# CAMMA-public/SelfPose3d

Hardware: AMD Instinct MI355X
Metric: multi-view samples/sec (5-view Panoptic, 80x80x20 voxel) (higher is better)
Workload: dtype f32

## Files before the change

include/sp3d.h:

```cpp
#ifndef SP3D_H
#define SP3D_H

#include <stdint.h>

#ifdef __cplusplus
extern "C" {
#endif

#define SP3D_ABI_VERSION 3
#define SP3D_MAX_VIEWS 16
#define SP3D_MAX_TOPK 32

#define SP3D_CAM_STRIDE 64
#define SP3D_CAM_R 0
#define SP3D_CAM_T 9
#define SP3D_CAM_F 12
#define SP3D_CAM_C 14
#define SP3D_CAM_K 16
#define SP3D_CAM_P 19
#define SP3D_CAM_A 21
#define SP3D_CAM_W0 27
#define SP3D_CAM_H0 28
#define SP3D_CAM_FLIP 29
#define SP3D_CAM_RXY 32
// ... 90 lines not shown
                                 const float *grid_size, int W_in, int H_in, void *stream);

int sp3d_unproject_one_bwd(const float *cam, const int32_t *sample_of, const float *centers, const uint8_t *valid,
                           const float *grad_cubes, int64_t grad_cube_stride, const uint16_t *pass_mask, float *grad_hm,
                           int B, int P, int V, int h, int w, int X, int Y, int Z, const float *grid_size, int W_in,
                           int H_in, void *stream);

int sp3d_unproject_one_bwd_det(const float *cam, const int32_t *sample_of, const float *centers, const uint8_t *valid,
                               const float *grad_cubes, int64_t grad_cube_stride, const uint16_t *pass_mask,
                               int64_t *grad_fixed, const float *scale, int B, int P, int V, int h, int w, int X, int Y,
                               int Z, const float *grid_size, int W_in, int H_in, void *stream);

int64_t sp3d_nms_topk_workspace_bytes(int B, int X, int Y, int Z, int k);
int sp3d_nms_topk(const float *root_cubes, int B, int X, int Y, int Z, int k, const float *grid_size,
                  const float *grid_center, float *vals, int64_t *idx, float *locs, void *workspace, void *stream);
int sp3d_nms_proposals(const float *root_cubes, int B, int X, int Y, int Z, int k, const float *grid_size,
                       const float *grid_center, float threshold, float *vals, int64_t *idx, float *locs,
                       float *grid_centers, void *workspace, void *stream);

int sp3d_soft_argmax(const float *x, const float *grids, float *out, int Bv, int J, int64_t N, float beta,
                     void *stream);
int sp3d_soft_argmax_grid(const float *x, const float *centers, const float *grid_size, int X, int Y, int Z,
                          float *out, int Bv, int J, float beta, void *stream);
int sp3d_soft_argmax_grid_train(const float *x, const float *centers, const float *grid_size, int X, int Y, int Z, float *out,
                                float *stats, int Bv, int J, float beta, void *stream);
int sp3d_soft_argmax_grid_bwd(const float *x, const float *centers, const float *grid_size, int X, int Y, int Z,
                              const float *out, const float *stats, const float *grad_out, float *grad_x, int Bv, int J,
                              float beta, void *stream);

int sp3d_channel_shift_act(float *y, const float *shift, const float *residual, int mode, int64_t batch, int C,
                           int64_t inner, int channels_last, void *stream);

int sp3d_fetch_ring(const float *ring, float *dst, uint32_t *counter, int R, int n, void *stream);

int sp3d_maxpool2x_cl(const float *x, float *y, int B, int X, int Y, int Z, int C, void *stream);

int sp3d_crop_shift_act_cl(const float *src, float *dst, const float *shift, int B, int C, int X, int Y, int Z, int SX, int SY,
                           int SZ, int relu, void *stream);

int sp3d_rfft3d(const float *in, float *out, int batch, int SX, int SY, int SZ, void *stream);
int sp3d_irfft3d(float *in, float *out, int batch, int SX, int SY, int SZ, void *stream);

int sp3d_cfft2d(float *data, int batch, int SX, int SY, int inverse, void *stream);
int sp3d_cfft2d_ex(float *data, int batch, int SX, int SY, int inverse, int rows_in, int rows_out, void *stream);

int sp3d_zdft_fwd_cl(const float *x, float *spec, int B, int C, int Cout, int X, int Y, int Z, int SX, int SY, int SZ,
                     void *stream);
int sp3d_zdft_inv_cl(const float *spec, float *y, const float *shift, int B, int O, int X, int Y, int Z, int SX, int SY, int SZ,
                     int relu, void *stream);

int sp3d_unproject_fwd_zdft(const float *const *hm_views, int Jp, const float *cam, const float *centers,
                            const uint8_t *valid, float *spec, int B, int V, int J, int h, int w, int X, int Y, int Z,
                            const float grid_size[3], int W_in, int H_in, int SZ, void *stream);
int sp3d_cfft2d_88_tiled(const float *tiled, float *planes, int batch, int X, int Y, void *stream);

int sp3d_freq_contract_ty(const float *X, const float *T, const float *tw, float *Y, int B, int C, int O, int rows, int SY,
                          void *stream);

int sp3d_gaussian_target_3d(const float *roots, int B, int R, const float *gx, const float *gy, const float *gz, int X,
                            int Y, int Z, float sigma, float *target, void *stream);
int sp3d_render_root_heatmaps(const float *roots, int B, int R, const float *cam, int V, int h, int w, float stride,
                              float *out, void *stream);
int sp3d_render_joints_fwd(const float *kps, const int *count, int N, int P, int J, int h, int w, float sigma, float *out,
                           void *stream);
int sp3d_render_joints_bwd(const float *kps, const int *count, const float *grad_out, int N, int P, int J, int h, int w,
                           float sigma, float *grad_kps, void *stream);

int sp3d_freq_contract(const float *X, const float *W, float *Y, int B, int C, int O, int64_t F, void *stream);
int sp3d_freq_contract_ex(const float *P, const float *Q, float *Y, int I, int J, int K, int64_t F, int64_t sPi,
                          int64_t sPk, int64_t sQj, int64_t sQk, int conj_p, int conj_q, void *stream);

int sp3d_wino_input(const float *x, float *V, int B, int X, int Y, int Z, int C, void *stream);
int sp3d_wino_output(const float *M, float *y, const float *shift, const float *residual, int mode, int B, int X, int Y,
                     int Z, int O, void *stream);
int sp3d_wino_fused(const float *x, const float *U, float *y, const float *shift, const float *residual, int mode, int B,
                    int X, int Y, int Z, int C, int O, void *stream);

int sp3d_wino_fused_split(const float *x, const void *U3, float *y, const float *shift, const float *residual, int mode, int B,
                          int X, int Y, int Z, int C, int O, void *stream);

int sp3d_wino_fused_split64(const float *x, const void *U3, float *y, const float *shift, const float *residual, int mode,
                            int B, int X, int Y, int Z, int C, int O, void *stream);

int sp3d_conv3_split(const float *x, const void *W3, float *y, const float *shift, const float *residual, int mode, int B,
                     int X, int Y, int Z, int C, int O, void *stream);


int sp3d_conv3_split_skip(const float *x, const void *W3, float *y, const float *shift, const float *xs, const void *WS,
                          int B, int X, int Y, int Z, int C, int O, int CS, void *stream);

int sp3d_wino_fused_split64_skip(const float *x, const void *U3, float *y, const float *shift, const float *xs, const void *WS,
                                 int B, int X, int Y, int Z, int C, int O, int CS, void *stream);

int sp3d_upsample2x_scatter(const float *G, float *out, const float *shift, const float *skip, int64_t batch, int X, int Y,
                            int Z, int O, void *stream);

int sp3d_upsample2x_scatter_head(const float *G, float *head, const float *shift, const float *skip, const float *wout,
                                 const float *bout, int64_t batch, int X, int Y, int Z, int O, int J, void *stream);

int sp3d_upconv2x_fused(const float *x, const void *w_split, const float *shift, const float *skip, const float *w_out,
                        const float *b_out, float *out, int64_t batch, int X, int Y, int Z, int CIN, int O, int J, void *stream);

#define SP3D_GBN_F32 0
#define SP3D_GBN_F64 1
#define SP3D_GBN_REPLICAS 16
#define SP3D_GBN_PLAIN 0
#define SP3D_GBN_RELU 1
#define SP3D_GBN_ADD_RELU 2
int64_t sp3d_gbn_workspace_bytes(int G, int C);
int sp3d_gbn_forward(const void *x, void *y, int dtype, const int32_t *group_of, const int32_t *group_samples, int N,
                     int64_t S, int C, int G, int G_update, const void *weight, const void *bias, void *running_mean,
                     void *running_var, double eps, double momentum, int mode, const void *residual, void *mean,
                     void *invstd, void *scale, void *shift, double *workspace, void *stream);
int sp3d_gbn_backward(const void *x, const void *dy, void *dx, int dtype, const int32_t *group_of,
                      const int32_t *group_samples, int N, int64_t S, int C, int G, const void *weight, const void *mean,
                      const void *invstd, const void *scale, const void *shift, int mode, const void *y,
                      void *grad_residual, void *grad_weight, void *grad_bias, void *k123, double *workspace, void *stream);

#ifdef __cplusplus
}
#endif
#endif
```

selfpose3d_amd/_lib.py:

```python
from __future__ import annotations

import ctypes as C
import os
from typing import Optional, Sequence

import torch

_HERE = os.path.dirname(os.path.abspath(__file__))
_DEFAULT_LIB_PATH = os.path.join(_HERE, "libsp3d.so")
NOPK_LIB_PATH = os.path.join(_HERE, "libsp3d_nopk.so")
LIB_PATH = os.environ.get("SP3D_LIB_PATH") or _DEFAULT_LIB_PATH

LAYOUT_PLANAR = 0
LAYOUT_NHWC = 1
OUT_CHANNELS_LAST = 0x100
HM_BF16 = 0x200
OUT_BF16 = 0x400
HM_ONE_CHANNEL = 0x800
HM_WIDE_MASK = 0x1000
SCATTER_AUTO, SCATTER_PER_TAP, SCATTER_MERGE = 0, 2, 3
SCATTER_WIDE = 0x100
MAX_VIEWS = 16
MAX_TOPK = 32
ABI_VERSION = 3
# ... 711 lines not shown
    Fn = 1
    for d in Pf.shape[2:]:
        Fn *= int(d)
    p0, p1, q0, q1 = int(Pf.shape[0]), int(Pf.shape[1]), int(Qf.shape[0]), int(Qf.shape[1])
    if mode == "fwd":
        I, K, J = p0, p1, q0
        sPi, sPk, sQj, sQk, cp, cq = p1 * Fn, Fn, q1 * Fn, Fn, 0, 1
        ok = q1 == p1
    elif mode == "dx":
        I, K, J = p0, p1, q1
        sPi, sPk, sQj, sQk, cp, cq = p1 * Fn, Fn, Fn, q1 * Fn, 0, 0
        ok = q0 == p1
    elif mode == "dw":
        I, K, J = p1, p0, q1
        sPi, sPk, sQj, sQk, cp, cq = Fn, p1 * Fn, Fn, q1 * Fn, 1, 0
        ok = q0 == p0
    else:
        raise Sp3dError(f"freq_contract_ex: unknown mode {mode}")
    if not ok:
        raise Sp3dError("freq_contract_ex: contracted dimensions differ")
    Y = torch.empty((I, J) + tuple(Pf.shape[2:]), dtype=torch.complex64, device=Pf.device)
    check(lib.sp3d_freq_contract_ex(Pf.data_ptr(), Qf.data_ptr(), Y.data_ptr(), I, J, K, Fn, sPi, sPk, sQj, sQk, cp, cq,
                                    _stream(Pf.device)), "sp3d_freq_contract_ex")
    return Y


_WINO_G = ((1.0, 0.0, 0.0), (0.5, 0.5, 0.5), (0.5, -0.5, 0.5), (0.0, 0.0, 1.0))


def wino_weights(w: torch.Tensor) -> torch.Tensor:
    G = torch.tensor(_WINO_G, dtype=torch.float64, device=w.device)
    u = torch.einsum("ai,bj,ck,ozijk->abczo", G, G, G, w.double())
    return u.reshape(64, w.shape[1], w.shape[0]).float().contiguous()


def wino_weights_split(U: torch.Tensor, chunk: int = 8) -> torch.Tensor:
    P, Cc, O = (int(v) for v in U.shape)
    U = U.float()
    hi = U.bfloat16()
    r = U - hi.float()
    mid = r.bfloat16()
    lo = (r - mid.float()).bfloat16()
    pieces = torch.stack([mid, hi, lo], 0).reshape(3, P, Cc // chunk, chunk // 4, 4, O)
    return pieces.permute(1, 2, 3, 5, 0, 4).contiguous()


def conv_weights_split(w: torch.Tensor) -> torch.Tensor:
    O, Cc = int(w.shape[0]), int(w.shape[1])
    taps = int(w.shape[2]) * int(w.shape[3]) * int(w.shape[4])
    pc = wino_weights_split(w.float().permute(4, 3, 2, 1, 0).reshape(taps, Cc, O).contiguous(), 8)
    mid, hi, lo = pc[..., 0, :], pc[..., 1, :], pc[..., 2, :]
    return torch.stack([hi, lo, hi, hi, mid, mid], -2).contiguous()


def conv_weights_split24(w: torch.Tensor) -> torch.Tensor:
    O, Cc = int(w.shape[0]), int(w.shape[1])
    pc = wino_weights_split(w.float().permute(4, 3, 2, 1, 0).reshape(27, Cc, O).contiguous(), 8)
    pc = pc.reshape(27, Cc // 8, 2, O // 32, 32, 3, 4).permute(0, 1, 3, 2, 4, 5, 6)
    hl = torch.stack([pc[..., 1, :], pc[..., 2, :]], -2).reshape(27, Cc // 8, O // 32, 512)
    mid = pc[..., 0, :].reshape(27, Cc // 8, O // 32, 256)
    return torch.cat([hl, mid], -1).contiguous()


def skip_fold_enabled() -> bool:
    return os.environ.get("SP3D_FOLD_SKIP", "1") not in ("0", "")


def _require_skip(xs: torch.Tensor, skip_w: torch.Tensor, x: torch.Tensor, CS: int, numel: int, who: str):
    _require_cl3d_f32(xs, who)
    if xs.device != x.device or tuple(xs.shape) != (x.shape[0], CS) + tuple(x.shape[2:]):
        raise Sp3dError(f"{who}: xs must be ({x.shape[0]}, {CS}, ...) on the grid and device of x, got {tuple(xs.shape)} on {xs.device}")
    if skip_w.device != x.device or skip_w.dtype != torch.bfloat16 or not skip_w.is_contiguous() or skip_w.numel() != numel:
        raise Sp3dError(f"{who}: skip_w must be the split records of the ({x.shape[1]}, {CS}, 1, 1, 1) weight on {x.device}; got "
                        f"{tuple(skip_w.shape)}, {skip_w.dtype}, {skip_w.device}, contiguous={skip_w.is_contiguous()}")


def conv3_split_(x: torch.Tensor, W3: torch.Tensor, shift: torch.Tensor, mode: int,
                 residual: Optional[torch.Tensor] = None, *, xs: Optional[torch.Tensor] = None,
                 skip_w: Optional[torch.Tensor] = None, out: Optional[torch.Tensor] = None) -> torch.Tensor:
    lib = load()
    _require_cuda(x, "x")
    B, Cc, X, Y, Z = (int(v) for v in x.shape)
    _require_cl3d_f32(x, "conv3_split_")
    O = int(W3.shape[3])
    dev = x.device
    y = _result_cl3d(out, B, O, X, Y, Z, x, "conv3_split_")
    if xs is not None or skip_w is not None:
        if xs is None or skip_w is None or int(mode) != 1 or residual is not None:
            raise Sp3dError("conv3_split_: the folded skip takes xs AND skip_w, mode 1 and no residual")
        CS = 16
        _require_skip(xs, skip_w, x, CS, CS * O * 6, "conv3_split_")
        check(lib.sp3d_conv3_split_skip(x.data_ptr(), W3.data_ptr(), y.data_ptr(), shift.data_ptr(), xs.data_ptr(),
                                        skip_w.data_ptr(), B, X, Y, Z, Cc, O, CS, _stream(dev)), "sp3d_conv3_split_skip")
        return y
    if residual is not None:
        residual = _as_cl3d(residual)
    check(lib.sp3d_conv3_split(x.data_ptr(), W3.data_ptr(), y.data_ptr(), shift.data_ptr(), _opt(residual), int(mode),
                               B, X, Y, Z, Cc, O, _stream(dev)), "sp3d_conv3_split")
    return y


def quarter_direct_enabled() -> bool:
    return os.environ.get("SP3D_QUARTER_DIRECT", "1") not in ("0", "")


def quarter_direct_covers(B: int, C: int, O: int, X: int, Y: int, Z: int) -> bool:
    blocks = B * (X // 5) * (Y // 5) * (Z // 5)
    return O == 128 and C in (64, 128) and X % 5 == 0 and Y % 5 == 0 and Z % 5 == 0 and blocks <= 64


def conv3_split128_(x: torch.Tensor, W3: torch.Tensor, shift: torch.Tensor, mode: int,
                    residual: Optional[torch.Tensor] = None, *, out: Optional[torch.Tensor] = None) -> torch.Tensor:
    lib = load()
    _require_cuda(x, "x")
    B, Cc, X, Y, Z = (int(v) for v in x.shape)
    _require_cl3d_f32(x, "conv3_split128_")
    O = 128
    if W3.device != x.device or W3.dtype != torch.bfloat16 or not W3.is_contiguous() or tuple(W3.shape) != (27, Cc // 8, O // 32, 768):
        raise Sp3dError(f"conv3_split128_: W3 must be conv_weights_split24 of the ({O}, {Cc}, 3, 3, 3) weight on {x.device}; got "
                        f"{tuple(W3.shape)}, {W3.dtype}, {W3.device}, contiguous={W3.is_contiguous()}")
    out = _result_cl3d(out, B, O, X, Y, Z, x, "conv3_split128_")
    if residual is not None:
        residual = _as_cl3d(residual)
    check(lib.sp3d_conv3_split(x.data_ptr(), W3.data_ptr(), out.data_ptr(), shift.data_ptr(), _opt(residual), int(mode),
                                  B, X, Y, Z, Cc, O, _stream(x.device)), "sp3d_conv3_split")
    return out


def wino_conv3d_(x: torch.Tensor, U: torch.Tensor, shift: torch.Tensor, mode: int,
                 residual: Optional[torch.Tensor] = None, *, direct: Optional[torch.Tensor] = None,
                 out: Optional[torch.Tensor] = None) -> torch.Tensor:
    lib = load()
    _require_cuda(x, "x")
    B, Cc, X, Y, Z = (int(v) for v in x.shape)
    _require_cl3d_f32(x, "wino_conv3d_")
    O = int(U.shape[2])
    if residual is not None:
        residual = _as_cl3d(residual)
    if direct is not None and quarter_direct_enabled() and quarter_direct_covers(B, Cc, O, X, Y, Z):
        return conv3_split128_(x, direct, shift, mode, residual, out=out)
    y = _result_cl3d(out, B, O, X, Y, Z, x, "wino_conv3d_")
    T = B * ((X + 1) // 2) * ((Y + 1) // 2) * ((Z + 1) // 2)
    V = torch.empty((64, T, Cc), dtype=torch.float32, device=x.device)
    check(lib.sp3d_wino_input(x.data_ptr(), V.data_ptr(), B, X, Y, Z, Cc, _stream(x.device)), "sp3d_wino_input")
    M = torch.bmm(V, U)
    check(lib.sp3d_wino_output(M.data_ptr(), y.data_ptr(), shift.data_ptr(), _opt(residual), int(mode), B, X, Y, Z, O,
                               _stream(x.device)), "sp3d_wino_output")
    return y


def wino_fused_conv3d_(x: torch.Tensor, U: torch.Tensor, shift: torch.Tensor, mode: int,
                       residual: Optional[torch.Tensor] = None, U3: Optional[torch.Tensor] = None, *,
                       xs: Optional[torch.Tensor] = None, skip_w: Optional[torch.Tensor] = None,
                       out: Optional[torch.Tensor] = None) -> torch.Tensor:
    lib = load()
    _require_cuda(x, "x")
    B, Cc, X, Y, Z = (int(v) for v in x.shape)
    _require_cl3d_f32(x, "wino_fused_conv3d_")
    O = int(U.shape[2])
    y = _result_cl3d(out, B, O, X, Y, Z, x, "wino_fused_conv3d_")
    if xs is not None or skip_w is not None:
        if xs is None or skip_w is None or U3 is None or int(mode) != 1 or residual is not None:
            raise Sp3dError("wino_fused_conv3d_: the folded skip takes U3, xs AND skip_w, mode 1 and no residual")
        CS = 32
        _require_skip(xs, skip_w, x, CS, CS * O * 3, "wino_fused_conv3d_")
        check(lib.sp3d_wino_fused_split64_skip(x.data_ptr(), U3.data_ptr(), y.data_ptr(), shift.data_ptr(), xs.data_ptr(),
                                               skip_w.data_ptr(), B, X, Y, Z, Cc, O, CS, _stream(x.device)),
              "sp3d_wino_fused_split64_skip")
        return y
    if residual is not None:
        residual = _as_cl3d(residual)
    if U3 is None:
        name, weights = "sp3d_wino_fused", U
    else:
        name, weights = ("sp3d_wino_fused_split64" if O == 64 else "sp3d_wino_fused_split"), U3
    check(getattr(lib, name)(x.data_ptr(), weights.data_ptr(), y.data_ptr(), shift.data_ptr(), _opt(residual), int(mode),
                             B, X, Y, Z, Cc, O, _stream(x.device)), name)
    return y


def upconv_weights_split(w_gemm: torch.Tensor) -> torch.Tensor:
    Cc, O = int(w_gemm.shape[0]), int(w_gemm.shape[1]) // 8
# ... 95 lines not shown
```

selfpose3d_amd/csrc/sp3d_conv3_direct.hip:

```cpp
#include <hip/hip_runtime.h>
#include <stdint.h>

#include "../../include/sp3d.h"
#include "sp3d_conv3_host.h"
#include "sp3d_split.h"

namespace sp3d {

constexpr int CD_BX = 16, CD_BY = 8, CD_BZ = 4;
constexpr int CD_RX = CD_BX + 2, CD_RY = CD_BY + 2, CD_RZ = CD_BZ + 2, CD_VOX = 8, CD_ROW = CD_RX * CD_VOX, CD_ZP = CD_RY * CD_ROW + 4;
constexpr int CD_PLANE = CD_RZ * CD_ZP;
constexpr int CD_BUF = 2 * CD_PLANE;
constexpr int CD_NV4 = CD_RX * CD_RY * CD_RZ * 2;
constexpr int CD_PROD = 4;
constexpr int CD_PER = (CD_NV4 + 64 * CD_PROD - 1) / (64 * CD_PROD);
constexpr int CD_BUFS = ((CD_BUF / 4 + 63) / 64) * 256;
#ifndef SP3D_WG_ABLATE
#define SP3D_WG_ABLATE 0
#endif
struct CdRec { u32x4 hl, hh, mm; };


#ifdef SP3D_CD_TIMELINE
__device__ unsigned long long *g_cd_tl = nullptr;
#define CD_STAMP(slot) do { __builtin_amdgcn_sched_barrier(0); if (g_cd_tl && blockIdx.x == 0 && lane == 0 && item < 64) { g_cd_tl[(wave * 64 + item) * 4 + (slot)] = __builtin_readcyclecounter(); \
     \
    if (wave == 0 && (slot) == 0 && item == 0) { g_cd_tl[(7 * 64 + 62) * 4 + 0] = wall_clock64(); g_cd_tl[(7 * 64 + 62) * 4 + 1] = __builtin_readcyclecounter(); } \
    if (wave == 0 && (slot) == 3) { g_cd_tl[(7 * 64 + 63) * 4 + 0] = wall_clock64(); g_cd_tl[(7 * 64 + 63) * 4 + 1] = __builtin_readcyclecounter(); } } __builtin_amdgcn_sched_barrier(0); } while (0)
#else
#define CD_STAMP(slot) do { (void)item; } while (0)
#endif

template <int C, int MODE, bool SKIP = false>
__global__ __launch_bounds__(64 * (4 + CD_PROD)) __attribute__((amdgpu_waves_per_eu(2, 2)))
void conv3_split_kernel(const float *__restrict__ x, const unsigned *__restrict__ W3, float *__restrict__ y,
                        const float *__restrict__ shift, const float *__restrict__ res, int B, int X, int Y, int Z, int NBX,
                        int NBY, int NBZ, int nblocks, const float *__restrict__ xs = nullptr,
                        const unsigned *__restrict__ WS = nullptr)
{
    constexpr int O = 32, NCH = C / 8, CS = 16;
    extern __shared__ __attribute__((aligned(16))) unsigned cd_lds[];
    const int tid = threadIdx.x, lane = tid & 63, wave = tid >> 6, t = lane & 31, h = lane >> 5;
    const int my_blocks = ((int)blockIdx.x < nblocks) ? (nblocks - 1 - (int)blockIdx.x) / (int)gridDim.x + 1 : 0;
    const int n_items = my_blocks * NCH;
    auto decode = [&](int item, int &b, int &ox0, int &oy0, int &oz0) {
        int bid = (int)blockIdx.x + (item / NCH) * (int)gridDim.x;
        const int bz = bid % NBZ; bid /= NBZ;
        const int by = bid % NBY; bid /= NBY;
        const int bx = bid % NBX;
        b = bid / NBX;
        ox0 = bx * CD_BX; oy0 = by * CD_BY; oz0 = bz * CD_BZ;
    };

    if (wave >= 4) {
        const int pt = tid - 256;
        __builtin_amdgcn_s_setprio(2);
        float4 d[CD_PER];
        int lo_[CD_PER], rel[CD_PER], vxyz[CD_PER];
#pragma unroll
        for (int u = 0; u < CD_PER; ++u) {
            const int idx = pt + 64 * CD_PROD * u;
            const int v = idx >> 1, half = idx & 1;
            const int vx = v % CD_RX, vy = (v / CD_RX) % CD_RY, vz = v / (CD_RX * CD_RY);
            lo_[u] = idx < CD_NV4 ? half * CD_PLANE + vz * CD_ZP + vy * CD_ROW + vx * CD_VOX : -1;
            rel[u] = ((vx * Y + vy) * Z + vz) * C + half * 4;
            vxyz[u] = idx < CD_NV4 ? (vx | (vy << 8) | (vz << 16)) : 0x00ffffff;
        }
        auto issue = [&](int k) {
            int b, ox0, oy0, oz0;
            decode(k, b, ox0, oy0, oz0);
            const int64_t vox0 = (((int64_t)b * X + (ox0 - 1)) * Y + (oy0 - 1)) * Z + (oz0 - 1);
            const float *xb = x + vox0 * C + (k % NCH) * 8;
            const int xlo = 1 - ox0, xhi = X + 1 - ox0, ylo = 1 - oy0, yhi = Y + 1 - oy0, zlo = 1 - oz0, zhi = Z + 1 - oz0;
#pragma unroll
            for (int u = 0; u < CD_PER; ++u) {
                const int vx = vxyz[u] & 255, vy = (vxyz[u] >> 8) & 255, vz = vxyz[u] >> 16;
                const bool in = vx >= xlo && vx < xhi && vy >= ylo && vy < yhi && vz >= zlo && vz < zhi;
                d[u] = make_float4(0.0f, 0.0f, 0.0f, 0.0f);
                if (in) d[u] = *reinterpret_cast<const float4 *>(xb + rel[u]);
            }
        };
        if (n_items > 0) issue(0);
        for (int k = 0; k <= n_items; ++k) {
            if (k < n_items) {
                { const int item = k; CD_STAMP(0); }
                unsigned *buf = cd_lds + (k & 1) * CD_BUFS;
#ifdef SP3D_CD_TIMELINE
                __builtin_amdgcn_s_waitcnt(0);
                { const int item = k; CD_STAMP(3); }
#endif
#pragma unroll
                for (int u = 0; u < CD_PER; ++u) {
                    u32x4 q0, q1;
                    split3(d[u], q0, q1);
                    if (lo_[u] >= 0) {
                        unsigned *p = buf + lo_[u];
                        *reinterpret_cast<u32x4 *>(p) = q0;
                        *reinterpret_cast<u32x4 *>(p + 4) = q1;
                    }
                }
                { const int item = k; CD_STAMP(1); }
                if (k + 1 < n_items) issue(k + 1);
            }
            if (k < n_items) { const int item = k; CD_STAMP(2); }
            __syncthreads();
        }
        return;
    }

    const int a_off = h * CD_PLANE + (t >> 3) * CD_ZP + (t & 7) * CD_ROW + 4 * wave * CD_VOX;
    const unsigned *wl = W3 + ((int64_t)h * O + t) * 12;
    struct W3Rec { CdRec d[3]; };
    auto load_w = [&](int q) {
        const int cc = (q / 9) % NCH, st = q % 9;
        const unsigned *r = wl + ((int64_t)(3 * st) * NCH + cc) * 2 * O * 12;
        W3Rec w;
#pragma unroll
        for (int dx = 0; dx < 3; ++dx) {
#if SP3D_W16_ABLATE & 2
            (void)r; w.d[dx].hl = u32x4{0x3f803f80u + (unsigned)q, 0x3f803f80u, 0x3f803f80u + (unsigned)dx, 0x3f803f80u};
            w.d[dx].hh = w.d[dx].hl ^ 0x00010001u; w.d[dx].mm = w.d[dx].hl ^ 0x00020002u;
#else
            w.d[dx].hl = *reinterpret_cast<const u32x4 *>(r + (int64_t)dx * NCH * 2 * O * 12);
            w.d[dx].hh = *reinterpret_cast<const u32x4 *>(r + (int64_t)dx * NCH * 2 * O * 12 + 4);
            w.d[dx].mm = *reinterpret_cast<const u32x4 *>(r + (int64_t)dx * NCH * 2 * O * 12 + 8);
#endif
        }
        return w;
    };
    struct Opnd { u32x4 lh[6], hm[6]; };
    f32x16 acc[4];
    W3Rec w0, w1;
    if (n_items > 0) w0 = load_w(0);
    __syncthreads();
    for (int k = 1; k <= n_items; ++k) {
        const int item = k - 1, cc = item % NCH;
        const unsigned *ab = cd_lds + (item & 1) * CD_BUFS + a_off;
        if (cc == 0) {
#pragma unroll
            for (int m = 0; m < 4; ++m)
#pragma unroll
                for (int v = 0; v < 16; ++v) acc[m][v] = 0.0f;
        }
        auto load_a = [&](int st, Opnd &a) {
            const int dz = st / 3, dy = st % 3;
#pragma unroll
            for (int j = 0; j < 6; ++j) {
                const unsigned *p = ab + dz * CD_ZP + dy * CD_ROW + j * CD_VOX;
                a.lh[j] = *reinterpret_cast<const u32x4 *>(p);
                a.hm[j] = *reinterpret_cast<const u32x4 *>(p + 4);
            }
        };
        Opnd a0, a1;
        load_a(0, a0);
        const int q0 = item * 9;
        float s0[4];
        unsigned so[4];
        CD_STAMP(0);
#pragma unroll
        for (int st = 0; st < 9; ++st) {
            if (SKIP && st == 8 && cc == NCH - 1) {
                int b, ox0, oy0, oz0;
                decode(item, b, ox0, oy0, oz0);
                const float *xb = xs + (int64_t)b * X * Y * Z * CS;
                const int ys = min(oy0 + (t & 7), Y - 1), zs = min(oz0 + (t >> 3), Z - 1);
#pragma unroll
                for (int i = 0; i < 4; ++i) {
                    const int xv = min(ox0 + 4 * wave + i, X - 1);
                    so[i] = (unsigned)(((xv * Y + ys) * Z + zs) * CS + 4 * h);
                    s0[i] = xb[so[i]];
                }
            }
            __builtin_amdgcn_sched_barrier(0);
            w1 = load_w(min(q0 + st + 1, n_items * 9 - 1));
            if (st + 1 < 9) load_a(st + 1, a1);
#pragma unroll
            for (int dx = 0; dx < 3; ++dx) {
#pragma unroll
                for (int i = 0; i < 4; ++i) acc[i] = mfma_bf16(a0.lh[i + dx], w0.d[dx].hl, acc[i]);
#pragma unroll
                for (int i = 0; i < 4; ++i) acc[i] = mfma_bf16(a0.hm[i + dx], w0.d[dx].hh, acc[i]);
#pragma unroll
                for (int i = 0; i < 4; ++i) acc[i] = mfma_bf16(a0.hm[i + dx], w0.d[dx].mm, acc[i]);
            }
#pragma unroll
            for (int r = 0; r < 12; ++r) {
                __builtin_amdgcn_sched_group_barrier(0x008, 1, 0);
                __builtin_amdgcn_sched_group_barrier(0x100, 1, 0);
            }
#pragma unroll
            for (int r = 0; r < 9; ++r) {
                __builtin_amdgcn_sched_group_barrier(0x008, 1, 0);
                __builtin_amdgcn_sched_group_barrier(0x020, 1, 0);
            }
            __builtin_amdgcn_sched_group_barrier(0x008, 15, 0);
            __builtin_amdgcn_sched_barrier(0);
            a0 = a1;
            w0 = w1;
        }
        CD_STAMP(1);
        if (SKIP && cc == NCH - 1) {
            float4 sv[2][4];
            {
                int b, ox0, oy0, oz0;
                decode(item, b, ox0, oy0, oz0);
                const float *xb = xs + (int64_t)b * X * Y * Z * CS;
#pragma unroll
                for (int i = 0; i < 4; ++i) {
                    const float *p = xb + so[i];
                    sv[0][i] = make_float4(s0[i], p[1], p[2], p[3]);
                    sv[1][i] = *reinterpret_cast<const float4 *>(p + 8);
                }
            }
            CdRec ws[2];
#pragma unroll
            for (int c2 = 0; c2 < 2; ++c2) {
                const unsigned *r = WS + (unsigned)(((c2 * 2 + h) * O + t) * 12);
                ws[c2].hl = *reinterpret_cast<const u32x4 *>(r);
                ws[c2].hh = *reinterpret_cast<const u32x4 *>(r + 4);
                ws[c2].mm = *reinterpret_cast<const u32x4 *>(r + 8);
            }
#pragma unroll
            for (int c2 = 0; c2 < 2; ++c2) {
                __builtin_amdgcn_sched_barrier(0);
                u32x4 lh[4], hm[4];
#pragma unroll
                for (int i = 0; i < 4; ++i) split3(sv[c2][i], lh[i], hm[i]);
#pragma unroll
                for (int i = 0; i < 4; ++i) acc[i] = mfma_bf16(lh[i], ws[c2].hl, acc[i]);
#pragma unroll
                for (int i = 0; i < 4; ++i) acc[i] = mfma_bf16(hm[i], ws[c2].hh, acc[i]);
#pragma unroll
                for (int i = 0; i < 4; ++i) acc[i] = mfma_bf16(hm[i], ws[c2].mm, acc[i]);
            }
        }
        if (cc == NCH - 1) {
            int b, ox0, oy0, oz0;
            decode(item, b, ox0, oy0, oz0);
            if (ox0 + CD_BX <= X && oy0 + CD_BY <= Y && oz0 + CD_BZ <= Z) {
                const float sh = shift[t];
                const int64_t obase = ((((int64_t)b * X + ox0 + 4 * wave) * Y + oy0 + 4 * h) * Z + oz0) * O + t;
#pragma unroll
                for (int i = 0; i < 4; ++i)
#pragma unroll
                    for (int v = 0; v < 16; ++v) {
                        const int64_t idx = obase + (((int64_t)i * Y + (v & 3)) * Z + (v >> 2)) * O;
                        float val = acc[i][v] + sh;
                        if (MODE == 2) val += res[idx];
                        if (MODE >= 1) val = SKIP ? relu_keep_nan(val) : fmaxf(val, 0.0f);
                        if (MODE == 3) val += res[idx];
#if SP3D_W16_ABLATE & 16
                        if (val == 123.456f)
#endif
                        y[idx] = val;
                    }
            } else {
            float *scr = reinterpret_cast<float *>(cd_lds + 2 * CD_BUFS) + wave * 1024;
            const int g = lane & 7;
            const float4 sh4 = *reinterpret_cast<const float4 *>(shift + 4 * g);
#pragma unroll
            for (int mb = 0; mb < 4; ++mb) {
#pragma unroll
                for (int v = 0; v < 16; ++v) scr[(8 * (v >> 2) + (v & 3) + 4 * h) * 32 + t] = acc[mb][v];
                __builtin_amdgcn_fence(__ATOMIC_RELEASE, "wavefront");
                __builtin_amdgcn_wave_barrier();
#pragma unroll
                for (int r = 0; r < 4; ++r) {
                    const int m = (lane >> 3) + 8 * r;
                    float4 a = *reinterpret_cast<const float4 *>(scr + m * 32 + 4 * g);
                    const int xo = ox0 + 4 * wave + mb, yo = oy0 + (m & 7), zo = oz0 + (m >> 3);
                    if (xo < X && yo < Y && zo < Z) {
                        const int64_t vox = (((int64_t)b * X + xo) * Y + yo) * Z + zo;
                        a.x += sh4.x; a.y += sh4.y; a.z += sh4.z; a.w += sh4.w;
                        float4 rr = make_float4(0.0f, 0.0f, 0.0f, 0.0f);
                        if (MODE >= 2) rr = *reinterpret_cast<const float4 *>(res + vox * O + 4 * g);
                        if (MODE == 2) { a.x += rr.x; a.y += rr.y; a.z += rr.z; a.w += rr.w; }
                        if (MODE >= 1 && SKIP) { a.x = relu_keep_nan(a.x); a.y = relu_keep_nan(a.y); a.z = relu_keep_nan(a.z); a.w = relu_keep_nan(a.w); }
                        if (MODE >= 1 && !SKIP) { a.x = fmaxf(a.x, 0.0f); a.y = fmaxf(a.y, 0.0f); a.z = fmaxf(a.z, 0.0f); a.w = fmaxf(a.w, 0.0f); }
                        if (MODE == 3) { a.x += rr.x; a.y += rr.y; a.z += rr.z; a.w += rr.w; }
#if SP3D_W16_ABLATE & 16
                        if (a.x == 123.456f)
#endif
                        *reinterpret_cast<float4 *>(y + vox * O + 4 * g) = a;
                    }
                }
                __builtin_amdgcn_fence(__ATOMIC_RELEASE, "wavefront");
                __builtin_amdgcn_wave_barrier();
            }
            }
        }
        CD_STAMP(2);
        __syncthreads();
        CD_STAMP(3);
    }
}


}


using namespace sp3d;

static int conv3_cu_count(int dev)
{
    static int cu_count[64] = {0};
    if (dev < 0 || dev >= 64) return 256;
    if (cu_count[dev] == 0) {
        int n = 0;
        cu_count[dev] = (hipDeviceGetAttribute(&n, hipDeviceAttributeMultiprocessorCount, dev) == hipSuccess && n > 0) ? n : 256;
    }
    return cu_count[dev];
}

template <int C, int MODE, bool SKIP>
static int conv3_split_launch(const float *x, const void *W3, float *y, const float *shift, const float *residual, const float *xs,
                              const void *WS, int B, int X, int Y, int Z, const Conv3Grid &g, void *stream)
{
    int dev = 0;
    { const hipError_t ed = hipGetDevice(&dev); if (ed != hipSuccess) return (int)ed; }
    const int cus = conv3_cu_count(dev);
    const int rounds = (int)((g.blocks + cus - 1) / cus);
    const int nwg = (int)((g.blocks + rounds - 1) / rounds);
    const size_t lds = (size_t)2 * CD_BUFS * sizeof(unsigned) + 4 * 1024 * sizeof(float);
    static bool attr_dev[64] = {};
    const int slot = (dev < 0 || dev >= 64) ? 63 : dev;
    if (!attr_dev[slot] || slot == 63) {
        const hipError_t ea = hipFuncSetAttribute(reinterpret_cast<const void *>(conv3_split_kernel<C, MODE, SKIP>),
                                                  hipFuncAttributeMaxDynamicSharedMemorySize, (int)lds);
        if (ea != hipSuccess) return (int)ea;
        attr_dev[slot] = true;
    }
    hipLaunchKernelGGL((conv3_split_kernel<C, MODE, SKIP>), dim3((unsigned)nwg), dim3(64 * (4 + CD_PROD)), lds, (hipStream_t)stream, x,
                       reinterpret_cast<const unsigned *>(W3), y, shift, residual, B, X, Y, Z, g.NBX, g.NBY, g.NBZ, (int)g.blocks, xs,
                       reinterpret_cast<const unsigned *>(WS));
    return launch_status();
}

extern "C" int sp3d_conv3_split(const float *x, const void *W3, float *y, const float *shift, const float *residual, int mode,
                                int B, int X, int Y, int Z, int C, int O, void *stream)
{
    if (O == 128) return conv3_split128(x, W3, y, shift, residual, mode, B, X, Y, Z, C, O, stream);
    const Conv3Grid g = conv3_grid(B, X, Y, Z, CD_BX, CD_BY, CD_BZ);
    const bool supported = O == 32 && (C == 16 || C == 32) && !((reinterpret_cast<uintptr_t>(W3) | reinterpret_cast<uintptr_t>(y)) & 15);
    const bool in_range = (int64_t)X * Y * Z * C * 2 <= 0x7fffffff && g.blocks <= 0x7fffffff;
    if (const int rc = conv3_check(B, X, Y, Z, mode, x && W3 && y && shift && (mode < 2 || residual), supported, in_range)) return rc;
    return with_mode(mode, [&](auto m) {
        constexpr int M = decltype(m)::value;
        return C == 16 ? conv3_split_launch<16, M, false>(x, W3, y, shift, residual, nullptr, nullptr, B, X, Y, Z, g, stream)
                       : conv3_split_launch<32, M, false>(x, W3, y, shift, residual, nullptr, nullptr, B, X, Y, Z, g, stream);
    });
}

extern "C" int sp3d_conv3_split_skip(const float *x, const void *W3, float *y, const float *shift, const float *xs,
                                     const void *WS, int B, int X, int Y, int Z, int C, int O, int CS, void *stream)
{
    const Conv3Grid g = conv3_grid(B, X, Y, Z, CD_BX, CD_BY, CD_BZ);
    const bool supported = O == 32 && C == 32 && CS == 16 &&
                           !((reinterpret_cast<uintptr_t>(W3) | reinterpret_cast<uintptr_t>(WS) | reinterpret_cast<uintptr_t>(xs) |
                              reinterpret_cast<uintptr_t>(y)) & 15);
    const bool in_range = (int64_t)X * Y * Z * C * 2 <= 0x7fffffff && g.blocks <= 0x7fffffff;
    if (const int rc = conv3_check(B, X, Y, Z, 1, x && W3 && y && shift && xs && WS, supported, in_range)) return rc;
    return conv3_split_launch<32, 1, true>(x, W3, y, shift, nullptr, xs, WS, B, X, Y, Z, g, stream);
}


extern "C" int sp3d_debug_conv3_timeline(void *dev_buffer)
{
#ifdef SP3D_CD_TIMELINE
    unsigned long long *p = (unsigned long long *)dev_buffer;
    return (int)hipMemcpyToSymbol(HIP_SYMBOL(sp3d::g_cd_tl), &p, sizeof(p));
#else
    (void)dev_buffer;
    return SP3D_EUNSUPPORTED;
#endif
}
```

selfpose3d_amd/v2v_net.py:

```python
from __future__ import annotations

from typing import NamedTuple, Optional

import torch
import torch.nn as nn
import torch.nn.functional as F


def _bn(c):
    from .grouped_bn import GroupedBatchNorm3d
    return GroupedBatchNorm3d(c)


def _grouped(bn, training: bool) -> bool:
    return training and getattr(bn, "groups", None) is not None


def fft_len(n: int) -> int:
    m = n + (n & 1)
    while True:
        r, odd = m, 0
        for q in (2, 3, 5, 7, 11, 13):
            if q > 2 and r % q == 0:
                odd += 1
# ... 167 lines not shown
        x = self.encoder_res1(F.max_pool3d(x, 2, 2))
        s2 = self.skip_res2(x)
        x = self.encoder_res2(F.max_pool3d(x, 2, 2))
        x = self.decoder_res2(self.mid_res(x))
        x = self.decoder_upsample2(x) + s2
        x = self.decoder_upsample1(self.decoder_res1(x)) + s1
        return x


class TiledZSpectrum:

    def __init__(self, spec: torch.Tensor, X: int, Y: int, Z: int, SZ: int):
        self.spec, self.X, self.Y, self.Z, self.SZ = spec, int(X), int(Y), int(Z), int(SZ)
        self.shape = (int(spec.shape[0]), int(spec.shape[1]), self.X, self.Y, self.Z)
        self.device, self.is_cuda, self.dtype = spec.device, spec.is_cuda, torch.float32


class _Conv(NamedTuple):
    w: torch.Tensor
    shift: torch.Tensor
    u: Optional[torch.Tensor] = None
    split: Optional[torch.Tensor] = None
    direct: Optional[torch.Tensor] = None


class _Res(NamedTuple):
    c1: _Conv
    c2: _Conv
    skip: Optional[torch.Tensor]
    skip_direct: Optional[torch.Tensor] = None
    skip_split: Optional[torch.Tensor] = None


class _Up(NamedTuple):
    wT: torch.Tensor
    shift: torch.Tensor
    wg: torch.Tensor
    split: Optional[torch.Tensor] = None


class _FoldedV2V:

    def __init__(self, net: "V2VNet"):
        self.net = net
        self.key = None
        self.layers = {}
        self.spectra = {}
        self.xpad = {}

    def graph_tensors(self):
        return dict(self.layers), dict(self.spectra), dict(self.xpad)

    @staticmethod
    def _key(net):
        ps = list(net.parameters()) + list(net.buffers())
        w3 = net.front_layers[1].res_branch[0].weight
        return (tuple((p.data_ptr(), p._version) for p in ps), str(w3.device), bool(is_cl(w3)))

    def _ensure_built(self):
        key = self._key(self.net)
        if key != self.key:
            self._build()
            self.key = key

    @staticmethod
    def _fold(conv, bn, transposed=False):
        s = bn.weight / torch.sqrt(bn.running_var + bn.eps)
        shape = (1, -1, 1, 1, 1) if transposed else (-1, 1, 1, 1, 1)
        w = conv.weight * s.view(shape)
        fmt = torch.channels_last_3d if is_cl(conv.weight) else torch.contiguous_format
        b = conv.bias if conv.bias is not None else torch.zeros_like(bn.running_mean)
        return w.contiguous(memory_format=fmt), ((b - bn.running_mean) * s + bn.bias).contiguous()

    @staticmethod
    def _conv3_record(w, shift):
        from . import _lib
        cout, cin = int(w.shape[0]), int(w.shape[1])
        routes = {conv3_route(cin, cout, (b, 2, 2, 2), True, ws, dc) for b in (1, 1 << 20) for ws in (True, False) for dc in (True, False)}
        if not w.is_cuda or routes == {"library"}:
            return _Conv(w, shift)
        u = _lib.wino_weights(w)
        split = _lib.wino_weights_split(u, 16 if cout == 64 else 8) if "wino_fused_conv3d_" in routes else None
        if "conv3_split_" in routes:
            direct = _lib.conv_weights_split(w)
        elif "wino_conv3d_" in routes and cout == 128 and cin in (64, 128):
            direct = _lib.conv_weights_split24(w)
        else:
            direct = None
        return _Conv(w, shift, u, split, direct)

    def _build(self):
        from . import _lib
        n, layers = self.net, {}
        layers["front"] = _Conv(*self._fold(n.front_layers[0].block[0], n.front_layers[0].block[1]))
        ed = n.encoder_decoder
        for name in ("front_res", "encoder_res1", "encoder_res2", "mid_res", "decoder_res2", "decoder_res1", "skip_res1",
                     "skip_res2"):
            blk = n.front_layers[1] if name == "front_res" else getattr(ed, name)
            w1, s1 = self._fold(blk.res_branch[0], blk.res_branch[1])
            w2, s2 = self._fold(blk.res_branch[3], blk.res_branch[4])
            ws = sd = sp = None
            if len(blk.skip_con) > 0:
                ws, ss = self._fold(blk.skip_con[0], blk.skip_con[1])
                s2 = (s2 + ss).contiguous()
                co, ci = int(ws.shape[0]), int(ws.shape[1])
                if ws.is_cuda and (co, ci) == (32, 16):
                    sd = _lib.conv_weights_split(ws)
                if ws.is_cuda and (co, ci) == (64, 32):
                    sp = _lib.wino_weights_split(ws.reshape(co, ci).t().reshape(1, ci, co).contiguous(), 16)
            layers[name] = _Res(self._conv3_record(w1, s1), self._conv3_record(w2, s2), ws, sd, sp)
        for name in ("decoder_upsample2", "decoder_upsample1"):
            blk = getattr(ed, name).block
            wT, sT = self._fold(blk[0], blk[1], transposed=True)
            wg = wT.permute(0, 2, 3, 4, 1).reshape(wT.shape[0], 8 * wT.shape[1]).contiguous()
            fused = wg.is_cuda and (int(wT.shape[0]), int(wT.shape[1])) in ((128, 64), (64, 32))
            layers[name] = _Up(wT, sT, wg, _lib.upconv_weights_split(wg) if fused else None)
        self.layers, self.spectra, self.xpad = layers, {}, {}

    def _route(self, x, c: "_Conv") -> str:
        n = self.net
        if c.u is None or not is_cl(x):
            return "library"
        return conv3_route(int(c.w.shape[1]), int(c.w.shape[0]), (x.shape[0],) + tuple(x.shape[2:]), n.winograd,
                           getattr(n, "wino_split", True), getattr(n, "direct_conv", True))

    def _conv3(self, x, c: "_Conv", mode, residual=None, xs=None, skip_w=None):
        from . import _lib
        route = self._route(x, c)
        split = getattr(self.net, "wino_split", True)
        if route == "conv3_split_":
            return _lib.conv3_split_(x, c.direct, c.shift, mode, residual, xs=xs, skip_w=skip_w)
        if route == "wino_fused_conv3d_":
            return _lib.wino_fused_conv3d_(x, c.u, c.shift, mode, residual, c.split if split else None, xs=xs, skip_w=skip_w)
        assert xs is None and skip_w is None, route
        if route == "wino_conv3d_":
            return _lib.wino_conv3d_(x, c.u, c.shift, mode, residual, direct=c.direct)
        return _lib.channel_shift_act_(F.conv3d(x, c.w, None, 1, 1), c.shift, mode, residual)

    def _folded_skip(self, x, h, r: "_Res"):
        from . import _lib
        if r.skip is None or not _lib.skip_fold_enabled() or not (is_cl(x) and x.is_cuda and x.dtype == torch.float32):
            return None
        route, widths = self._route(h, r.c2), (int(r.c2.w.shape[1]), int(r.c2.w.shape[0]), int(x.shape[1]))
        if route == "conv3_split_" and widths == (32, 32, 16):
            return r.skip_direct
        if route == "wino_fused_conv3d_" and getattr(self.net, "wino_split", True) and widths == (64, 64, 32):
            return r.skip_split
        return None

    def _res(self, x, name):
        r = self.layers[name]
        h = self._conv3(x, r.c1, 1)
        if r.skip is None:
            return self._conv3(h, r.c2, 2, x)
        rec = self._folded_skip(x, h, r)
        if rec is not None:
            return self._conv3(h, r.c2, 1, xs=x, skip_w=rec)
        return self._conv3(h, r.c2, 2, self._conv1(x, r.skip))

    _tuned_shapes: "set[tuple]" = set()
    _tune_gemms = None

    @staticmethod
    def _tunable():
        import os
        on = _FoldedV2V._tune_gemms
        if on is None:
# ... 293 lines not shown
```

Baseline: 2785.

## Use compact 24-byte split weight records in full-resolution direct conv3 kernel

```diff
diff --git a/include/sp3d.h b/include/sp3d.h
--- a/include/sp3d.h
+++ b/include/sp3d.h
@@ -196,6 +196,7 @@
 int sp3d_wino_fused_split64(const float *x, const void *U3, float *y, const float *shift, const float *residual, int mode,
                             int B, int X, int Y, int Z, int C, int O, void *stream);
 
+#define SP3D_CONV3_W24 0x100
 int sp3d_conv3_split(const float *x, const void *W3, float *y, const float *shift, const float *residual, int mode, int B,
                      int X, int Y, int Z, int C, int O, void *stream);
 
diff --git a/selfpose3d_amd/_lib.py b/selfpose3d_amd/_lib.py
--- a/selfpose3d_amd/_lib.py
+++ b/selfpose3d_amd/_lib.py
@@ -817,7 +817,13 @@
     _require_cuda(x, "x")
     B, Cc, X, Y, Z = (int(v) for v in x.shape)
     _require_cl3d_f32(x, "conv3_split_")
-    O = int(W3.shape[3])
+    if W3.dim() == 6 and tuple(W3.shape[:3]) + tuple(W3.shape[4:]) == (27, Cc // 8, 2, 6, 4):
+        O, w24 = int(W3.shape[3]), 0
+    elif W3.dim() == 4 and tuple(W3.shape) == (27, Cc // 8, 1, 768) and W3.dtype == torch.bfloat16 and W3.is_contiguous():
+        O, w24 = 32 * int(W3.shape[2]), CONV3_W24
+    else:
+        raise Sp3dError(f"conv3_split_: W3 must be conv_weights_split(w), (27, {Cc // 8}, 2, O, 6, 4), or conv_weights_split24(w), "
+                        f"(27, {Cc // 8}, 1, 768), of the (O, {Cc}, 3, 3, 3) weight; got {tuple(W3.shape)}")
     dev = x.device
     y = _result_cl3d(out, B, O, X, Y, Z, x, "conv3_split_")
     if xs is not None or skip_w is not None:
@@ -826,13 +832,22 @@
         CS = 16
         _require_skip(xs, skip_w, x, CS, CS * O * 6, "conv3_split_")
         check(lib.sp3d_conv3_split_skip(x.data_ptr(), W3.data_ptr(), y.data_ptr(), shift.data_ptr(), xs.data_ptr(),
-                                        skip_w.data_ptr(), B, X, Y, Z, Cc, O, CS, _stream(dev)), "sp3d_conv3_split_skip")
+                                        skip_w.data_ptr(), B, X, Y, Z, Cc, O, CS | w24, _stream(dev)), "sp3d_conv3_split_skip")
         return y
     if residual is not None:
         residual = _as_cl3d(residual)
-    check(lib.sp3d_conv3_split(x.data_ptr(), W3.data_ptr(), y.data_ptr(), shift.data_ptr(), _opt(residual), int(mode),
+    if int(mode) > 0 and int(mode) & CONV3_W24:
+        raise Sp3dError(f"conv3_split_: the layout flag comes from the shape of W3, not from mode ({mode})")
+    check(lib.sp3d_conv3_split(x.data_ptr(), W3.data_ptr(), y.data_ptr(), shift.data_ptr(), _opt(residual), int(mode) | w24,
                                B, X, Y, Z, Cc, O, _stream(dev)), "sp3d_conv3_split")
     return y
+
+
+CONV3_W24 = 0x100
+
+
+def fullres_w24_enabled() -> bool:
+    return os.environ.get("SP3D_FULLRES_W24", "1") not in ("0", "")
 
 
 def quarter_direct_enabled() -> bool:
diff --git a/selfpose3d_amd/csrc/sp3d_conv3_direct.hip b/selfpose3d_amd/csrc/sp3d_conv3_direct.hip
--- a/selfpose3d_amd/csrc/sp3d_conv3_direct.hip
+++ b/selfpose3d_amd/csrc/sp3d_conv3_direct.hip
@@ -31,7 +31,7 @@
 #define CD_STAMP(slot) do { (void)item; } while (0)
 #endif
 
-template <int C, int MODE, bool SKIP = false>
+template <int C, int MODE, bool SKIP = false, bool W24 = false>
 __global__ __launch_bounds__(64 * (4 + CD_PROD)) __attribute__((amdgpu_waves_per_eu(2, 2)))
 void conv3_split_kernel(const float *__restrict__ x, const unsigned *__restrict__ W3, float *__restrict__ y,
                         const float *__restrict__ shift, const float *__restrict__ res, int B, int X, int Y, int Z, int NBX,
@@ -110,11 +110,29 @@
 
     const int a_off = h * CD_PLANE + (t >> 3) * CD_ZP + (t & 7) * CD_ROW + 4 * wave * CD_VOX;
     const unsigned *wl = W3 + ((int64_t)h * O + t) * 12;
-    struct W3Rec { CdRec d[3]; };
+    struct W3Rec48 { CdRec d[3]; };
+    struct W24Tap { u32x4 hl; u32x2 m; };
+    struct W3Rec24 { W24Tap d[3]; };
+    using W3Rec = std::conditional_t<W24, W3Rec24, W3Rec48>;
+    const unsigned *wl24 = W3 + (h * 32 + t) * 4;
     auto load_w = [&](int q) {
         const int cc = (q / 9) % NCH, st = q % 9;
+        W3Rec w;
+        if constexpr (W24) {
+            const unsigned *r = wl24 + ((3 * st) * NCH + cc) * 384;
+#pragma unroll
+            for (int dx = 0; dx < 3; ++dx) {
+#if SP3D_W16_ABLATE & 2
+                (void)r; w.d[dx].hl = u32x4{0x3f803f80u + (unsigned)q, 0x3f803f80u, 0x3f803f80u + (unsigned)dx, 0x3f803f80u};
+                w.d[dx].m = u32x2{w.d[dx].hl.x ^ 0x00020002u, 0x3f813f80u};
+#else
+                w.d[dx].hl = *reinterpret_cast<const u32x4 *>(r + dx * NCH * 384);
+                w.d[dx].m = *reinterpret_cast<const u32x2 *>(r + dx * NCH * 384 + 256 - (h * 32 + t) * 2);
+#endif
+            }
+            return w;
+        } else {
         const unsigned *r = wl + ((int64_t)(3 * st) * NCH + cc) * 2 * O * 12;
-        W3Rec w;
 #pragma unroll
         for (int dx = 0; dx < 3; ++dx) {
 #if SP3D_W16_ABLATE & 2
@@ -127,6 +145,7 @@
 #endif
         }
         return w;
+        }
     };
     struct Opnd { u32x4 lh[6], hm[6]; };
     f32x16 acc[4];
@@ -172,6 +191,37 @@
                 }
             }
             __builtin_amdgcn_sched_barrier(0);
+            if constexpr (W24) {
+                auto tap = [&](int dx) {
+                    const u32x4 hl = w0.d[dx].hl;
+                    const u32x6 hb = {hl.x, hl.y, hl.x, hl.y, hl.z, hl.w};
+                    const u32x4 mm = {w0.d[dx].m.x, w0.d[dx].m.y, w0.d[dx].m.x, w0.d[dx].m.y};
+#pragma unroll
+                    for (int i = 0; i < 4; ++i) acc[i] = mfma_bf16(a0.lh[i + dx], split3_q1(hb), acc[i]);
+#pragma unroll
+                    for (int i = 0; i < 4; ++i) acc[i] = mfma_bf16(a0.hm[i + dx], split3_q0(hb), acc[i]);
+#pragma unroll
+                    for (int i = 0; i < 4; ++i) acc[i] = mfma_bf16(a0.hm[i + dx], mm, acc[i]);
+                };
+                w1 = load_w(min(q0 + st + 1, n_items * 9 - 1));
+                tap(0);
+#pragma unroll
+                for (int r = 0; r < 6; ++r) {
+                    __builtin_amdgcn_sched_group_barrier(0x008, 1, 0);
+                    __builtin_amdgcn_sched_group_barrier(0x020, 1, 0);
+                }
+                __builtin_amdgcn_sched_group_barrier(0x008, 6, 0);
+                __builtin_amdgcn_sched_barrier(0);
+                if (st + 1 < 9) load_a(st + 1, a1);
+                tap(1);
+#pragma unroll
+                for (int r = 0; r < 12; ++r) {
+                    __builtin_amdgcn_sched_group_barrier(0x008, 1, 0);
+                    __builtin_amdgcn_sched_group_barrier(0x100, 1, 0);
+                }
+                __builtin_amdgcn_sched_barrier(0);
+                tap(2);
+            } else {
             w1 = load_w(min(q0 + st + 1, n_items * 9 - 1));
             if (st + 1 < 9) load_a(st + 1, a1);
 #pragma unroll
@@ -194,6 +244,7 @@
                 __builtin_amdgcn_sched_group_barrier(0x020, 1, 0);
             }
             __builtin_amdgcn_sched_group_barrier(0x008, 15, 0);
+            }
             __builtin_amdgcn_sched_barrier(0);
             a0 = a1;
             w0 = w1;
@@ -312,7 +363,7 @@
     return cu_count[dev];
 }
 
-template <int C, int MODE, bool SKIP>
+template <int C, int MODE, bool SKIP, bool W24>
 static int conv3_split_launch(const float *x, const void *W3, float *y, const float *shift, const float *residual, const float *xs,
                               const void *WS, int B, int X, int Y, int Z, const Conv3Grid &g, void *stream)
 {
@@ -325,12 +376,12 @@
     static bool attr_dev[64] = {};
     const int slot = (dev < 0 || dev >= 64) ? 63 : dev;
     if (!attr_dev[slot] || slot == 63) {
-        const hipError_t ea = hipFuncSetAttribute(reinterpret_cast<const void *>(conv3_split_kernel<C, MODE, SKIP>),
+        const hipError_t ea = hipFuncSetAttribute(reinterpret_cast<const void *>(conv3_split_kernel<C, MODE, SKIP, W24>),
                                                   hipFuncAttributeMaxDynamicSharedMemorySize, (int)lds);
         if (ea != hipSuccess) return (int)ea;
         attr_dev[slot] = true;
     }
-    hipLaunchKernelGGL((conv3_split_kernel<C, MODE, SKIP>), dim3((unsigned)nwg), dim3(64 * (4 + CD_PROD)), lds, (hipStream_t)stream, x,
+    hipLaunchKernelGGL((conv3_split_kernel<C, MODE, SKIP, W24>), dim3((unsigned)nwg), dim3(64 * (4 + CD_PROD)), lds, (hipStream_t)stream, x,
                        reinterpret_cast<const unsigned *>(W3), y, shift, residual, B, X, Y, Z, g.NBX, g.NBY, g.NBZ, (int)g.blocks, xs,
                        reinterpret_cast<const unsigned *>(WS));
     return launch_status();
@@ -339,6 +390,8 @@
 extern "C" int sp3d_conv3_split(const float *x, const void *W3, float *y, const float *shift, const float *residual, int mode,
                                 int B, int X, int Y, int Z, int C, int O, void *stream)
 {
+    const bool w24 = mode >= 0 && (mode & SP3D_CONV3_W24);
+    if (w24) mode &= ~SP3D_CONV3_W24;
     if (O == 128) return conv3_split128(x, W3, y, shift, residual, mode, B, X, Y, Z, C, O, stream);
     const Conv3Grid g = conv3_grid(B, X, Y, Z, CD_BX, CD_BY, CD_BZ);
     const bool supported = O == 32 && (C == 16 || C == 32) && !((reinterpret_cast<uintptr_t>(W3) | reinterpret_cast<uintptr_t>(y)) & 15);
@@ -346,21 +399,27 @@
     if (const int rc = conv3_check(B, X, Y, Z, mode, x && W3 && y && shift && (mode < 2 || residual), supported, in_range)) return rc;
     return with_mode(mode, [&](auto m) {
         constexpr int M = decltype(m)::value;
-        return C == 16 ? conv3_split_launch<16, M, false>(x, W3, y, shift, residual, nullptr, nullptr, B, X, Y, Z, g, stream)
-                       : conv3_split_launch<32, M, false>(x, W3, y, shift, residual, nullptr, nullptr, B, X, Y, Z, g, stream);
+        if (w24)
+            return C == 16 ? conv3_split_launch<16, M, false, true>(x, W3, y, shift, residual, nullptr, nullptr, B, X, Y, Z, g, stream)
+                           : conv3_split_launch<32, M, false, true>(x, W3, y, shift, residual, nullptr, nullptr, B, X, Y, Z, g, stream);
+        return C == 16 ? conv3_split_launch<16, M, false, false>(x, W3, y, shift, residual, nullptr, nullptr, B, X, Y, Z, g, stream)
+                       : conv3_split_launch<32, M, false, false>(x, W3, y, shift, residual, nullptr, nullptr, B, X, Y, Z, g, stream);
     });
 }
 
 extern "C" int sp3d_conv3_split_skip(const float *x, const void *W3, float *y, const float *shift, const float *xs,
                                      const void *WS, int B, int X, int Y, int Z, int C, int O, int CS, void *stream)
 {
+    const bool w24 = CS >= 0 && (CS & SP3D_CONV3_W24);
+    if (w24) CS &= ~SP3D_CONV3_W24;
     const Conv3Grid g = conv3_grid(B, X, Y, Z, CD_BX, CD_BY, CD_BZ);
     const bool supported = O == 32 && C == 32 && CS == 16 &&
                            !((reinterpret_cast<uintptr_t>(W3) | reinterpret_cast<uintptr_t>(WS) | reinterpret_cast<uintptr_t>(xs) |
                               reinterpret_cast<uintptr_t>(y)) & 15);
     const bool in_range = (int64_t)X * Y * Z * C * 2 <= 0x7fffffff && g.blocks <= 0x7fffffff;
     if (const int rc = conv3_check(B, X, Y, Z, 1, x && W3 && y && shift && xs && WS, supported, in_range)) return rc;
-    return conv3_split_launch<32, 1, true>(x, W3, y, shift, nullptr, xs, WS, B, X, Y, Z, g, stream);
+    return w24 ? conv3_split_launch<32, 1, true, true>(x, W3, y, shift, nullptr, xs, WS, B, X, Y, Z, g, stream)
+               : conv3_split_launch<32, 1, true, false>(x, W3, y, shift, nullptr, xs, WS, B, X, Y, Z, g, stream);
 }
 
 
diff --git a/selfpose3d_amd/v2v_net.py b/selfpose3d_amd/v2v_net.py
--- a/selfpose3d_amd/v2v_net.py
+++ b/selfpose3d_amd/v2v_net.py
@@ -273,7 +273,7 @@
         u = _lib.wino_weights(w)
         split = _lib.wino_weights_split(u, 16 if cout == 64 else 8) if "wino_fused_conv3d_" in routes else None
         if "conv3_split_" in routes:
-            direct = _lib.conv_weights_split(w)
+            direct = _lib.conv_weights_split24(w) if _lib.fullres_w24_enabled() else _lib.conv_weights_split(w)
         elif "wino_conv3d_" in routes and cout == 128 and cin in (64, 128):
             direct = _lib.conv_weights_split24(w)
         else:
```

New measurement: 2774. Within noise of the previous version (-0.4%).
